# ISAE-PNX/SaDVIO

Measured on AMD Instinct MI355X. Metric: BA iterations/sec (ms/solve in ms_per_solve), 20-KF/8k-landmark window, higher is better.
Workload: dtype f64; 1 GPU; synthetic 20 KF x 8000 landmarks x 40000 reprojection factors (pixel), GN 10 iters (LM step attempts, early exits disabled); windows_per_gpu=1, parallelism=single window, n_kf=20, n_lmk=8000, n_obs=40000, reduced_dim=114

## Files before the change

sadvio_amd/csrc/ba_types.h:

```cpp
#pragma once
#include <stdint.h>

namespace sadvio {

struct SolveOpts {
    int max_num_iterations;
    int jacobi_scaling;
    int max_num_consecutive_invalid_steps;
    int pad;
    double function_tolerance, gradient_tolerance, parameter_tolerance;
    double initial_radius, max_radius, min_radius;
    double min_lm_diagonal, max_lm_diagonal, min_relative_decrease;
    double huber_a;
    double max_time_ticks;
};

struct WinDev {
    int n_kf, n_cam, n_lmk, n_obs;
    int kf_base, cam_base, lmk_base, obs_base;
    int n_free_kf, dpf, Np, Npose;
    long long S_off;
    int red_off;
    int tile_begin, tile_end;
    int prior_begin, prior_end;
// ... 80 lines not shown
    double radius, decrease_factor, x_cost, x_norm, initial_cost;
    int cur;
    int done, termination, iter;
    int n_success, n_unsuccess, n_invalid, pad;
};

struct FinalRec {
    LmState s;
    double fixed_cost;
};

struct IterAcc {
    double lin_cost;
    double cand_cost;
    double mcc;
    double step_norm2;
    double cand_norm2;
    double fixed_cost;
    unsigned long long gmax_bits;
    int chol_fail;
    int time_up;
};

struct TileAcc {
    double lin_cost, fixed_cost, gmax;
    double cand_cost, mcc, step_norm2, cand_norm2;
    double pad;
};

constexpr int BUILD_THREADS = 256;
constexpr int BUILD_WAVES = BUILD_THREADS / 64;
constexpr int MAX_TILE_KF = 24;
constexpr int MAX_TILE_FREE_KF = 20;
constexpr int MAX_GEMM_FREE_KF = 5;
constexpr int MAX_WIN_CAM = 8;
constexpr int STAGE_VALS = 18;
constexpr int MAX_LMK_OBS = 64;
constexpr int SOLVE_THREADS = 512;
constexpr int SOLVE_KFC_STRIDE = 32;
constexpr int SOLVE_KFC = 32;
constexpr int PRIOR_LIN = 28;
constexpr int PRE_KF = 8;
constexpr int PRE_MAX_TILES = 1024;
constexpr int MAX_LDS_NP = 174;

}
```

sadvio_amd/csrc/kernels.h:

```cpp
#pragma once
#include "ba_types.h"
#include "device_math.h"
#include "chol16.h"

namespace sadvio {

struct DevPtrs {
    const WinDev* win;
    const Tile* tiles;
    const double* kf_T0;
    const int* kf_fidx;
    double* xp; double* xv; double* xba; double* xbg;
    long long xp_stride, xv_stride, xl_stride;
    const double* kf_vel; const double* kf_ba; const double* kf_bg;
    const double* cam_K; const double* cam_T; const double* cam_isig;
    const double* lmk_p; double* xl; double* s_lmk;
    const unsigned char* lmk_const;
    const int* lmk_ob; const int* lmk_oe;
    const int* obs_kf; const int* obs_cam; const double* obs_meas;
    const unsigned char* obs_slot;
    const int* tile_kf;
    const int* tile_lmk;
    const int* tile_row;
    const int4* pre_lane;
// ... 421 lines not shown
    const Tile T = tiles[blockIdx.x];
    const int tid = threadIdx.x;
    if (tid < BUILD_THREADS / 8) {
        const int lane0 = tid * 8, wv = lane0 >> 6, ln = lane0 & 63;
        const int G = T.G, lpw = 64 / G, grp = ln / G, q0 = ln - grp * G, nl = T.n_lmk;
        const bool valid = wv * lpw + grp < nl;
        const int gl = nl > 0 ? tile_landmark(T, tile_lmk, valid ? wv * lpw + grp : 0) : T.lmk0;
        const int ob = nl > 0 ? lmk_ob[gl] : 0, nobs = (valid && nl > 0) ? lmk_oe[gl] - ob : 0;
        pre_lane[(long long)blockIdx.x * (BUILD_THREADS / 8) + tid] = make_int4(gl, ob, nobs | (valid ? 1 << 16 : 0), q0);
    }
    if (tid < PRE_KF) {
        int2 e = make_int2(-1, -1);
        if (tid < T.n_kf) { e.x = tile_kf[T.kf_off + tid]; e.y = kf_fidx[e.x]; }
        pre_kf[(long long)blockIdx.x * PRE_KF + tid] = e;
    }
}

template <bool COST_ONLY> __device__ __forceinline__ void pose_factor_eval(const DevPtrs& P, int slot, int idx, int ln);
template <int FACTOR, bool RARE, bool IMU>
__global__ __launch_bounds__(BUILD_THREADS, IMU ? 1 : 2) void k_build(DevPtrs P, int slot, int max_tile_kf, int strip_doubles, int Rp) {
    extern __shared__ __attribute__((aligned(16))) char smem[];
    if (IMU && (int)blockIdx.x >= P.n_tiles) {
        pose_factor_eval<false>(P, slot, (int)blockIdx.x - P.n_tiles, threadIdx.x);
        return;
    }
    const Tile T = P.tiles[blockIdx.x];
    const int tid = threadIdx.x, wv = tid >> 6, ln = tid & 63;
    int4 pl = make_int4(0, -1, 0, 0);
    int2 pk = make_int2(-1, -1);
    if (P.pre_lane) {
        pl = P.pre_lane[(long long)blockIdx.x * (BUILD_THREADS / 8) + (tid >> 3)];
        pk = P.pre_kf[(long long)blockIdx.x * PRE_KF + tid / POSE_TAB];
    }
    SADVIO_TS(3, 32);
    SADVIO_WG_TS(3, 0);
    __shared__ double s_part[BUILD_WAVES * 4];
    double* poseTab = (double*)smem;
    double* camTab = poseTab + (size_t)max_tile_kf * POSE_TAB;
    int* rowTab = (int*)(camTab + MAX_WIN_CAM * 17);
    double* stage = (double*)(smem + tile_tables_bytes(max_tile_kf));
    const int G = T.G, lpw = 64 / G;
    const int grp = ln / G, q = ln - grp * G;
    const int nl = T.n_lmk;
    LmState st;
    IterAcc a;
    LmState prev;
    const bool own_decision = !(slot == 0 || P.decide_kernel);
    double pc = 0.0, pm = 0.0, psn = 0.0, pcn = 0.0;
    auto decision_inputs = [&](int dec_w, int t0, int nt) {
        if (!own_decision) {
            st = P.states[(long long)dec_w * P.state_stride + slot];
            return;
        }
        a = P.acc[(long long)dec_w * P.state_stride + slot - 1];
        prev = P.states[(long long)dec_w * P.state_stride + slot - 1];
        if (P.world > 1) {
            if (wv == 0) {
                const double* rs = P.rank_s + (long long)dec_w * P.world * 4;
                for (int r = ln; r < P.world; r += 64) { pc += rs[4 * r]; pm += rs[4 * r + 1]; psn += rs[4 * r + 2]; pcn += rs[4 * r + 3]; }
            }
        } else {
            const TileAcc* ta = P.tacc + (long long)((slot - 1) & 1) * P.n_tiles + t0;
            double v[4][4];
#pragma unroll
            for (int u = 0; u < 4; u++) {
                const int t = tid + u * BUILD_THREADS;
                const bool in = t < nt;
                const TileAcc* e = ta + (in ? t : 0);
                v[u][0] = in ? e->cand_cost : 0.0; v[u][1] = in ? e->mcc : 0.0; v[u][2] = in ? e->step_norm2 : 0.0; v[u][3] = in ? e->cand_norm2 : 0.0;
            }
            pc = (v[0][0] + v[1][0]) + (v[2][0] + v[3][0]); pm = (v[0][1] + v[1][1]) + (v[2][1] + v[3][1]);
            psn = (v[0][2] + v[1][2]) + (v[2][2] + v[3][2]); pcn = (v[0][3] + v[1][3]) + (v[2][3] + v[3][3]);
        }
    };
    if (P.n_win == 1) decision_inputs(0, 0, P.n_tiles);
    else decision_inputs(T.w, T.win_tile0, T.win_ntiles);
    bool first_valid;
    int gl_first, pre_ob, pre_oe, pre_o;
    if (P.pre_lane) {
        first_valid = (pl.z >> 16) & 1; gl_first = pl.x; pre_ob = pl.y; pre_oe = pl.y + (pl.z & 0xff);
        pre_o = (pl.w + (tid & 7) < (pl.z & 0xff)) ? pl.y + pl.w + (tid & 7) : -1;
    } else {
        first_valid = wv * lpw + grp < nl;
        gl_first = tile_landmark(T, P.tile_lmk, first_valid ? wv * lpw + grp : 0);
        pre_ob = P.lmk_ob[gl_first]; pre_oe = P.lmk_oe[gl_first];
        pre_o = (first_valid && q < pre_oe - pre_ob) ? pre_ob + q : -1;
    }
    const int pre_lcode = P.lmk_const ? P.lmk_const[gl_first] : 0;
    double pre_p[3], pre_x0[3], pre_x1[3];
#pragma unroll
    for (int i = 0; i < 3; i++) {
        pre_p[i] = P.lmk_p[3 * (long long)gl_first + i];
        pre_x0[i] = P.xl[3 * (long long)gl_first + i];
        pre_x1[i] = P.xl[P.xl_stride + 3 * (long long)gl_first + i];
    }
    double pre_t0 = 0.0, pre_t1 = 0.0;
    if (P.pre_lane) {
        if (pk.x >= 0) {
            const long long src = (long long)pk.x * POSE_TAB + (tid - (tid / POSE_TAB) * POSE_TAB);
            pre_t0 = P.ptab[src]; pre_t1 = P.ptab[P.ptab_stride + src];
        }
    } else if (tid < T.n_kf * POSE_TAB) {
        const int k = tid / POSE_TAB, e = tid - k * POSE_TAB;
        const long long src = (long long)P.tile_kf[T.kf_off + k] * POSE_TAB + e;
        pre_t0 = P.ptab[src]; pre_t1 = P.ptab[P.ptab_stride + src];
    }
    for (int i = tid; i < T.n_cam * 17; i += blockDim.x) {
        const int c = i / 17, e = i - 17 * c;
        const int gc = T.cam_base + c;
        camTab[i] = e < 4 ? P.cam_K[4 * (long long)gc + e] : (e < 16 ? P.cam_T[12 * (long long)gc + e - 4] : P.cam_isig[gc]);
    }
    for (int i = tid; i < T.n_kf; i += blockDim.x) rowTab[i] = P.tile_row[T.kf_off + i];
    ObsPre pre_obs;
    pre_obs.slot = 0; pre_obs.craw = 0; pre_obs.m[0] = pre_obs.m[1] = pre_obs.m[2] = 0.0;
    if (pre_o >= 0) pre_obs = obs_prefetch<FACTOR>(P, pre_o);
    if (own_decision) {
        pc = wave_sum(pc); pm = wave_sum(pm); psn = wave_sum(psn); pcn = wave_sum(pcn);
        if (ln == 0) { s_part[wv * 4] = pc; s_part[wv * 4 + 1] = pm; s_part[wv * 4 + 2] = psn; s_part[wv * 4 + 3] = pcn; }
        __syncthreads();
        a.cand_cost += (s_part[0] + s_part[4]) + (s_part[8] + s_part[12]); a.mcc += (s_part[1] + s_part[5]) + (s_part[9] + s_part[13]);
        a.step_norm2 += (s_part[2] + s_part[6]) + (s_part[10] + s_part[14]); a.cand_norm2 += (s_part[3] + s_part[7]) + (s_part[11] + s_part[15]);
        st = lm_decide(prev, a, P.o);
        __syncthreads();
        if (T.first_of_window && tid == 0) { P.states[(long long)T.w * P.state_stride + slot] = st; trace_write(P, T.w, slot - 1, prev, a, st); }
    }
    if (st.done) return;
    SADVIO_TS(3, 33);
    double* Stile = stage + BUILD_WAVES * strip_doubles;
    const int Nt = 6 * T.n_free;
    const int tri_n = Nt * (Nt + 1) / 2;
    double* gT = Stile + tri_n;
    double* gfT = gT + Nt;
    double* hdT = gfT + Nt;
    const bool lds_mode = T.lds_mode != 0;
    if (tid < T.n_kf * POSE_TAB) poseTab[tid] = st.cur ? pre_t1 : pre_t0;
    {
        const double* src = P.ptab + (long long)st.cur * P.ptab_stride;
        for (int i = tid + blockDim.x; i < T.n_kf * POSE_TAB; i += blockDim.x) {
            const int k = i / POSE_TAB, e = i - k * POSE_TAB;
            poseTab[i] = src[(long long)P.tile_kf[T.kf_off + k] * POSE_TAB + e];
        }
    }
    if (lds_mode) {
        const int nz = tri_n + 3 * Nt;
        for (int i = tid; i < nz; i += blockDim.x) Stile[i] = 0.0;
    }
    __syncthreads();

    SADVIO_TS(3, 34);
    double* Sg = P.S + T.S_off;
    double* gredg = P.gred + T.red_off;
    double* gfullg = P.gfull + T.red_off;
    double* hdg = P.hdiag + T.red_off;
    const int dpf = T.dpf, Np = T.Np;
    const double* xl = P.xl + (long long)st.cur * P.xl_stride;
    double* wstage = stage + wv * strip_doubles;
    const bool gemm_mode = T.lds_mode == 2;
    double cost_part = 0.0, fixed_part = 0.0, gmax_part = 0.0;
    typedef double d4 __attribute__((ext_vector_type(4)));
    d4 accs[3] = {(d4){0.0, 0.0, 0.0, 0.0}, (d4){0.0, 0.0, 0.0, 0.0}, (d4){0.0, 0.0, 0.0, 0.0}};
    for (int base = wv * lpw; base < nl; base += BUILD_WAVES * lpw) {
        const int lm = base + grp;
        const bool lmk_valid = lm < nl;
        const bool first = base == wv * lpw;
        const int gl = first ? gl_first : tile_landmark(T, P.tile_lmk, lmk_valid ? lm : 0);
        const int ob = first ? pre_ob : P.lmk_ob[gl], oe = first ? pre_oe : P.lmk_oe[gl];
        const int nobs = lmk_valid ? oe - ob : 0;
        const int lcode = first ? pre_lcode : (P.lmk_const ? P.lmk_const[gl] : 0);
        const bool lfree = lcode == 0;
        ObsLin L;
        L.valid = q < nobs;
        L.row = -1; L.slot = 0; L.counted = false;
        if (L.valid) {
            double pw[3];
            ObsPre obq;
            if (first) {
#pragma unroll
                for (int i = 0; i < 3; i++) pw[i] = pre_p[i] + (st.cur ? pre_x1[i] : pre_x0[i]);
// ... 174 lines not shown
                    for (int j = 0; j < 6; j++) {
                        const int col = pb + j;
                        if (col > row) continue;
                        const double v = c0 * Jpb[j] + c1 * Jpb[6 + j];
                        if (lds_mode) atomic_add_f64(&Stile[tri(row, col)], v);
                        else atomic_add_f64(&Sg[s_index(T.ld, (pa / 6) * dpf + i, (pb / 6) * dpf + j)], v);
                    }
                }
            }
        }
        wave_lds_fence();
    }
        }
    if (gemm_mode && wv * lpw < nl) {
        const int lr = ln & 15, lk = ln >> 4;
        const int nt16 = (Nt + 15) >> 4;
#pragma unroll
        for (int pp = 0; pp < 3; pp++) {
            const int tr = pp < 1 ? 0 : 1, tc = pp - tr;
            if (tr < nt16) {
                const int col = 16 * tc + lr;
#pragma unroll
                for (int rg = 0; rg < 4; rg++) {
                    const int row = 16 * tr + lk + 4 * rg;
                    if (row < Nt && col <= row) atomic_add_f64(&Stile[tri(row, col)], -accs[pp][rg]);
                }
            }
        }
    }
    SADVIO_TS(3, 40);
    const double c = wave_sum(cost_part), f = wave_sum(fixed_part), gm = wave_max(gmax_part);
    if (ln == 0) { s_part[wv * 4] = c; s_part[wv * 4 + 1] = f; s_part[wv * 4 + 2] = gm; }
    __syncthreads();
    if (tid == 0) {
        double cs = 0.0, fs = 0.0, gs = 0.0;
        for (int k = 0; k < BUILD_WAVES; k++) { cs += s_part[k * 4]; fs += s_part[k * 4 + 1]; gs = fmax(gs, s_part[k * 4 + 2]); }
        TileAcc* ta = P.tacc + (long long)(slot & 1) * P.n_tiles + blockIdx.x;
        ta->lin_cost = cs; ta->fixed_cost = fs; ta->gmax = gs;
    }
    SADVIO_TS(3, 41);
    if (lds_mode) {
        int* growTab = (int*)stage;
        for (int k = tid; k < T.n_kf; k += blockDim.x) {
            const int r = rowTab[k];
            if (r >= 0) {
                const int fi = P.kf_fidx[P.tile_kf[T.kf_off + k]];
#pragma unroll
                for (int i = 0; i < 6; i++) growTab[r + i] = fi * dpf + i;
            }
        }
        __syncthreads();
        if (T.ld) {
            for (int row = wv; row < Nt; row += BUILD_WAVES) {
                const long long grow = (long long)growTab[row] * T.ld;
                const double* srow = Stile + tri(row, 0);
                for (int col = ln; col <= row; col += 64) {
                    const double v = srow[col];
                    if (v != 0.0) atomic_add_f64(&Sg[grow + growTab[col]], v);
                }
            }
        } else {
            for (int col = wv; col < Nt; col += BUILD_WAVES) {
                const int gc = growTab[col];
                for (int row = col + ln; row < Nt; row += 64) {
                    const double v = Stile[tri(row, col)];
                    if (v != 0.0) atomic_add_f64(&Sg[c16_index(growTab[row], gc)], v);
                }
            }
        }
        for (int i = tid; i < Nt; i += blockDim.x) {
            const int row = growTab[i];
            if (gT[i] != 0.0) atomic_add_f64(&gredg[row], gT[i]);
            if (gfT[i] != 0.0) atomic_add_f64(&gfullg[row], gfT[i]);
            if (hdT[i] != 0.0) atomic_add_f64(&hdg[row], hdT[i]);
        }
    }
    SADVIO_TS(3, 42);
    SADVIO_WG_TS(3, 1);
}

__device__ __forceinline__ double rsqrt_nr(double d) {
    double y = __builtin_amdgcn_rsq(d);
    const double t = d * y;
    const double e = __builtin_fma(-t, y, 1.0);
    const double p = __builtin_fma(0.375, e, 0.5);
    const double q = e * p;
    return __builtin_fma(y, q, y);
}

__device__ __forceinline__ double readlane_f64(double v, int lane) {
    int lo = __double2loint(v), hi = __double2hiint(v);
    lo = __builtin_amdgcn_readlane(lo, lane);
    hi = __builtin_amdgcn_readlane(hi, lane);
    return __hiloint2double(hi, lo);
}

constexpr int NBP = 6;

template <int NB>
__device__ __forceinline__ void factor_pivot(double (&Lk)[NB][NB], double (&Li)[NB][NB], bool& bad) {
#pragma unroll
    for (int j = 0; j < NB; j++) {
        double d = Lk[j][j];
#pragma unroll
        for (int q = 0; q < j; q++) d -= Lk[j][q] * Lk[j][q];
        if (!(d > 0.0) || !isfinite(d)) bad = true;
        double inv = rsqrt_nr(d);
        Lk[j][j] = d * inv;
        Li[j][j] = inv;
// ... 299 lines not shown
}

__device__ __noinline__ bool sparse_eval(const DevPtrs& P, const WinDev& W, const SparseDev& f, const double* xp, const double* xv,
                                        const double* xba, const double* xbg, const double* xl, const double* y,
                                        double* r, double* J) {
    return sparse_eval_t<false>(P, W, f, xp, xv, xba, xbg, xl, y, r, J);
}


__device__ __forceinline__ double prior_lin_record(const double* T0, const double* Tp, const double* inf, const double* d6, double* rec) {
    double r[6], J[36];
    pose_prior_factor(T0, Tp, inf, d6, r, J);
    double c = 0.0;
#pragma unroll
    for (int a = 0; a < 6; a++) {
        c += r[a] * r[a];
        double g = 0.0;
#pragma unroll
        for (int q = 0; q < 6; q++) g += J[6 * q + a] * r[q];
        rec[a] = g;
#pragma unroll
        for (int b = 0; b <= a; b++) {
            double hh = 0.0;
#pragma unroll
            for (int q = 0; q < 6; q++) hh += J[6 * q + a] * J[6 * q + b];
            rec[6 + a * (a + 1) / 2 + b] = hh;
        }
    }
    rec[27] = c;
    return c;
}

__device__ __noinline__ void pose_table_store(const double* T0, double d0, double d1, double d2, double d3, double d4, double d5, double* dst) {
    double T0r[12], tab[POSE_TAB];
#pragma unroll
    for (int i = 0; i < 12; i++) T0r[i] = T0[i];
    const double d6[6] = {d0, d1, d2, d3, d4, d5};
    pose_table_entry(T0r, d6, tab);
#pragma unroll
    for (int i = 0; i < POSE_TAB; i++) dst[i] = tab[i];
}
__device__ __noinline__ double prior_lin_record_call(const double* T0, double d0, double d1, double d2, double d3, double d4, double d5, const PriorDev* pr,
                                                     double* rec) {
    double T0r[12];
#pragma unroll
    for (int i = 0; i < 12; i++) T0r[i] = T0[i];
    const double d6[6] = {d0, d1, d2, d3, d4, d5};
    const PriorDev q = *pr;
    return prior_lin_record(T0r, q.T_prior, q.inf, d6, rec);
}

template <int MODE, bool EXTRAS>
__global__ __launch_bounds__(SOLVE_THREADS) void k_solve(DevPtrs P, int slot) {
    extern __shared__ __attribute__((aligned(16))) char smem[];
    constexpr bool BIG = MODE != 0;
    const int w = blockIdx.x;
    const WinDev W = P.win[w];
    if (BIG != (W.ld != 0)) return;
    const int tid = threadIdx.x;
    const int wv = __builtin_amdgcn_readfirstlane(tid >> 6), ln = tid & 63, nwv = blockDim.x >> 6;
    LmState* stp = P.states + (long long)w * P.state_stride + slot;
    IterAcc* acc = P.acc + (long long)w * P.state_stride + slot;
    __shared__ int s_done;
    __shared__ double s_red[SOLVE_THREADS / 64 * 4];
    SADVIO_TS(3, 0);
#ifdef SADVIO_KERNEL_TS
// ... 66 lines not shown
        c_y = gredg[tid]; c_gf = gfullg[tid]; c_hd = hdg[tid];
        if (slot != 0) c_sp = sp[tid];
    }
    const bool kf_pre = MODE == 0 && tid < W.n_kf && tid < SOLVE_KFC;
    int kf_fi = -1;
    double kf_t6[6], kf_t12[12], kf_vbb[9] = {0.0, 0.0, 0.0, 0.0, 0.0, 0.0, 0.0, 0.0, 0.0};
    if (kf_pre) {
        const int g = W.kf_base + tid;
        kf_fi = P.kf_fidx[g];
#pragma unroll
        for (int i = 0; i < 6; i++) kf_t6[i] = xp[6 * (long long)g + i];
#pragma unroll
        for (int i = 0; i < 12; i++) kf_t12[i] = P.kf_T0[12 * (long long)g + i];
        if (W.dpf == 15) {
            const double* xs3[3] = {P.xv + (long long)cur * P.xv_stride, P.xba + (long long)cur * P.xv_stride, P.xbg + (long long)cur * P.xv_stride};
#pragma unroll
            for (int q = 0; q < 3; q++)
#pragma unroll
                for (int i = 0; i < 3; i++) kf_vbb[3 * q + i] = xs3[q][3 * (long long)g + i];
        }
    }
    if (P.world > 1) {
        const double* rb = P.rank_b + (long long)w * P.world * 4;
        for (int r = tid; r < P.world; r += blockDim.x) { early_cost += rb[4 * r]; early_fixed += rb[4 * r + 1]; early_gm = fmax(early_gm, rb[4 * r + 2]); }
    } else {
        const TileAcc* ta = P.tacc + (long long)(slot & 1) * P.n_tiles + W.tile_begin;
        for (int t = tid; t < W.tile_end - W.tile_begin; t += blockDim.x) {
            early_cost += ta[t].lin_cost; early_fixed += ta[t].fixed_cost; early_gm = fmax(early_gm, ta[t].gmax);
        }
    }
    if (!BIG) {
        if (tid < Np) {
            y[tid] = c_y; gf[tid] = c_gf; hd[tid] = c_hd;
            gredg[tid] = 0.0; gfullg[tid] = 0.0; hdg[tid] = 0.0;
        }
        if (kf_pre) {
            double* c = kfc + tid * SOLVE_KFC_STRIDE;
            c[0] = (double)kf_fi;
#pragma unroll
            for (int i = 0; i < 6; i++) c[1 + i] = kf_t6[i];
#pragma unroll
            for (int i = 0; i < 12; i++) c[7 + i] = kf_t12[i];
            if (W.dpf == 15) {
#pragma unroll
                for (int i = 0; i < 9; i++) c[19 + i] = kf_vbb[i];
            }
        }
    }
    __syncthreads();
    SADVIO_TS(3, 1);
    if (det) {
        for (int p = 0; p < n_pri; p++) {
            const int fi = P.kf_fidx[P.priors[W.prior_begin + p].kf];
            if (tid < 28) {
                const double v = plin[p * PRIOR_LIN + tid];
                if (tid == 27) { if (fi < 0) fixed_part += v; else cost_part += v; }
                else if (fi >= 0) {
                    const int base = fi * W.dpf;
                    if (tid < 6) { y[base + tid] += v; gf[base + tid] += v; }
                    else {
                        const int q = tid - 6;
                        const int a = (int)((__builtin_sqrtf((float)(8 * q + 1)) - 1.0f) * 0.5f);
                        const int b = q - ((a * (a + 1)) >> 1);
                        A[aidx(base + a, base + b)] += v;
                        if (a == b) hd[base + a] += v;
                    }
                }
// ... 160 lines not shown
            if (slot == 0) { s = P.o.jacobi_scaling ? 1.0 / (1.0 + sqrt(hdi)) : 1.0; sp[tid] = s; }
            const double s2 = s * s;
            A[c16_index(tid, tid)] += fmin(fmax(s2 * hdi, P.o.min_lm_diagonal), P.o.max_lm_diagonal) / st.radius / s2;
            A[c16_index(Np, tid)] = y[tid];
        }
    } else {
        for (int i = tid; i < Np; i += blockDim.x) gm = fmax(gm, fabs(gf[i]));
    }
    gm = wave_max(gm); cost_part = wave_sum(cost_part); fixed_part = wave_sum(fixed_part);
    if (ln == 0) { s_red[wv * 3] = gm; s_red[wv * 3 + 1] = cost_part; s_red[wv * 3 + 2] = fixed_part; }
    if (tid == 0) s_done = 0;
    __syncthreads();
    if (!BIG) c16_symmetrize(A, nbt);
    if (tid == blockDim.x - 1) {
        double g = 0, cs = 0, fs = 0;
        for (int k = 0; k < nwv; k++) { g = fmax(g, s_red[k * 3]); cs += s_red[k * 3 + 1]; fs += s_red[k * 3 + 2]; }
        acc->gmax_bits = (unsigned long long)__double_as_longlong(g);
        acc->lin_cost = cs;
        acc->fixed_cost = fs;
        acc->cand_cost = 0.0; acc->mcc = 0.0; acc->step_norm2 = 0.0; acc->cand_norm2 = 0.0;
        const bool time_up = P.o.max_time_ticks > 0.0 && P.t_start && (double)(wall_clock64() - *P.t_start) >= P.o.max_time_ticks;
        acc->time_up = time_up ? 1 : 0;
        const bool no_iterations = st.iter == 0 && P.o.max_num_iterations <= 0;
        if (time_up || g <= P.o.gradient_tolerance || no_iterations) {
            LmState e = st;
            e.done = 1; e.termination = (time_up || g > P.o.gradient_tolerance) ? 0 : 3;
            e.x_cost = 0.5 * cs;
            if (e.iter == 0) e.initial_cost = e.x_cost;
            *stp = e;
            s_done = 1;
        }
    }
    __syncthreads();
    if (s_done) return;
    SADVIO_TS(3, 2);
    if (BIG) {
        for (int i = tid; i < Np; i += blockDim.x) {
            double s;
            if (slot == 0) { s = P.o.jacobi_scaling ? 1.0 / (1.0 + sqrt(hd[i])) : 1.0; sp[i] = s; }
            else s = sp[i];
            double s2 = s * s;
            A[aidx(i, i)] += fmin(fmax(s2 * hd[i], P.o.min_lm_diagonal), P.o.max_lm_diagonal) / st.radius / s2;
        }
        __syncthreads();
    }
    SADVIO_TS(3, 3);
    if (MODE == 1) return;
    }
    long long* ts = SADVIO_TS_PTR((P.debug & 4096) && blockIdx.x == 0 && slot == 3);
    if (MODE == 0) {
        bool ok = true;
        if (Np > 0) ok = c16_solve<1>(A, Np, xs, pub, yv, ts ? ts + 64 : nullptr);
        if (!ok) {
            if (tid == 0) acc->chol_fail = 1;
            return;
        }
    } else {
        y = P.delta + W.red_off;
        if (P.big_info[w] != 0) {
            for (int i = tid; i < Np; i += blockDim.x) { gredg[i] = 0.0; gfullg[i] = 0.0; hdg[i] = 0.0; }
            if (tid == 0) acc->chol_fail = 1;
            return;
        }
    }
    SADVIO_TS(3, 4);
    double* dl = P.delta + W.red_off;
    double sn = 0.0, cn = 0.0;
    bool bad = false;
    for (int i = tid; i < Np; i += blockDim.x) {
        double d = -xs[i];
        dl[i] = d;
        y[i] = d;
        sn += d * d;
        if (!isfinite(d)) bad = true;
        if (BIG) { gredg[i] = 0.0; gfullg[i] = 0.0; hdg[i] = 0.0; }
    }
    __syncthreads();
    SADVIO_TS(3, 5);
    double* xpc = P.xp + (long long)(1 - cur) * P.xp_stride;
    for (int k = tid; k < W.n_kf; k += blockDim.x) {
        int g = W.kf_base + k;
        const bool pre = MODE == 0 && k < SOLVE_KFC;
        const double* kc = kfc + (pre ? k : 0) * SOLVE_KFC_STRIDE;
        int fi = pre ? (int)kc[0] : P.kf_fidx[g];
        double d6[6];
        const double* T0r = pre ? kc + 7 : P.kf_T0 + 12 * (long long)g;
        double vbb[9];
        if (W.dpf == 15) {
            const double* xs3[3] = {P.xv + (long long)cur * P.xv_stride, P.xba + (long long)cur * P.xv_stride, P.xbg + (long long)cur * P.xv_stride};
#pragma unroll
            for (int q = 0; q < 3; q++)
#pragma unroll
                for (int i = 0; i < 3; i++) vbb[3 * q + i] = pre ? kc[19 + 3 * q + i] : xs3[q][3 * (long long)g + i];
        }
#pragma unroll
        for (int i = 0; i < 6; i++) {
            double v = (pre ? kc[1 + i] : xp[6 * (long long)g + i]) + (fi < 0 ? 0.0 : y[fi * W.dpf + i]);
            xpc[6 * (long long)g + i] = v;
            d6[i] = v;
            if (fi >= 0) cn += v * v;
        }
        pose_table_store(T0r, d6[0], d6[1], d6[2], d6[3], d6[4], d6[5], P.ptab + (long long)(1 - cur) * P.ptab_stride + (long long)g * POSE_TAB);
        if (W.dpf == 15) {
            double* xs3[3] = {P.xv + (long long)(1 - cur) * P.xv_stride, P.xba + (long long)(1 - cur) * P.xv_stride, P.xbg + (long long)(1 - cur) * P.xv_stride};
#pragma unroll
            for (int q = 0; q < 3; q++)
#pragma unroll
                for (int i = 0; i < 3; i++) {
                    const double v = vbb[3 * q + i] + (fi < 0 ? 0.0 : y[fi * 15 + 6 + 3 * q + i]);
                    xs3[q][3 * (long long)g + i] = v;
                    if (fi >= 0) cn += v * v;
                }
        }
// ... 70 lines not shown
            double jr[15], cd[15];
#pragma unroll
            for (int a = 0; a < 15; a++) { jr[a] = sc[q * 15 + a]; cd[a] = sc[SPARSE_COL + a]; }
            const double r = sc[225 + q];
            double m = 0.0;
#pragma unroll
            for (int a = 0; a < 15; a++) { const int ca = (int)cd[a]; if (ca >= 0) m += jr[a] * y[ca]; }
            mcc += -m * (r + 0.5 * m);
        }
    }
    if (EXTRAS && W.lobs_end > W.lobs_begin) {
        const int rows = W.factor_type == 0 ? 4 : 2;
        for (int it = tid; it < (W.lobs_end - W.lobs_begin) * 4; it += blockDim.x) {
            const int k = it >> 2, q = it & 3;
            if (q >= rows) continue;
            const LineObsDev& ob = P.lobs[W.lobs_begin + k];
            const int fi = P.kf_fidx[ob.kf], lc = P.lines[ob.line].col;
            if (fi < 0 && lc < 0) continue;
            const double* sc = P.line_scratch + (long long)(W.lobs_begin + k) * LINE_ROW;
            double m = 0.0;
            for (int a = 0; a < 6; a++) {
                if (fi >= 0) m += sc[q * 12 + a] * y[fi * W.dpf + a];
                if (lc >= 0) m += sc[q * 12 + 6 + a] * y[lc + a];
            }
            mcc += -m * (sc[48 + q] + 0.5 * m);
        }
    }
    SADVIO_TS(3, 7);
    sn = wave_sum(sn); cn = wave_sum(cn); mcc = wave_sum(mcc); cc = wave_sum(cc);
    if (bad) acc->chol_fail = 1;
    __syncthreads();
    if (ln == 0) { s_red[wv * 4] = sn; s_red[wv * 4 + 1] = cn; s_red[wv * 4 + 2] = mcc; s_red[wv * 4 + 3] = cc; }
    __syncthreads();
    if (tid == 0) {
        double a0 = 0, a1 = 0, a2 = 0, a3 = 0;
        for (int k = 0; k < nwv; k++) { a0 += s_red[k * 4]; a1 += s_red[k * 4 + 1]; a2 += s_red[k * 4 + 2]; a3 += s_red[k * 4 + 3]; }
        acc->step_norm2 = a0; acc->cand_norm2 = a1; acc->mcc = a2; acc->cand_cost = a3;
    }
    SADVIO_TS(3, 8);
    if (ts && tid == 0) { ts[15] = wall_clock64(); ts[21] = clock64(); }
}


__device__ __forceinline__ void zero_s_slice(const DevPtrs& P, const Tile& T, int tile_index) {
    if (T.ld != 0) return;
    const int n2 = c16_size(T.Np) >> 1;
    const int per = (n2 + T.win_ntiles - 1) / T.win_ntiles;
    const int i0 = (tile_index - T.win_tile0) * per, i1 = min(i0 + per, n2);
    double2* S2 = (double2*)(P.S + T.S_off);
    const double2 z2 = make_double2(0.0, 0.0);
    for (int i = i0 + (int)threadIdx.x; i < i1; i += blockDim.x) S2[i] = z2;
}

template <int FACTOR, bool RARE, bool IMU>
__global__ __launch_bounds__(BUILD_THREADS) void k_backsub(DevPtrs P, int slot, int max_tile_kf) {
    extern __shared__ __attribute__((aligned(16))) char smem[];
    if (IMU && (int)blockIdx.x >= P.n_tiles) {
        if (threadIdx.x < 64) pose_factor_eval<true>(P, slot, (int)blockIdx.x - P.n_tiles, threadIdx.x);
        return;
    }
    const Tile T = P.tiles[blockIdx.x];
    const int tid = threadIdx.x, wv = tid >> 6, ln = tid & 63;
    int4 pl = make_int4(0, -1, 0, 0);
    int2 pk = make_int2(-1, -1), pk6 = make_int2(-1, -1);
    if (P.pre_lane) {
        pl = P.pre_lane[(long long)blockIdx.x * (BUILD_THREADS / 8) + (tid >> 3)];
// ... 1117 lines not shown
```

sadvio_amd/csrc/solve_driver.h:

```cpp
#pragma once
#include <cstddef>
#include <type_traits>

#include "ba_handle.h"

namespace {

DevPtrs make_ptrs(sadvio_ba_handle* h, const SolveOpts& o, int state_stride) {
    DevPtrs P{};
    P.win = h->d_win.p; P.tiles = h->d_tiles.p;
    P.kf_T0 = h->d_kf_T0.p; P.kf_fidx = h->d_kf_fidx.p;
    P.xp = h->d_xp.p; P.xv = h->d_xv.p; P.xba = h->d_xba.p; P.xbg = h->d_xbg.p;
    P.xp_stride = 6LL * h->n_kf_tot; P.xv_stride = 3LL * h->n_kf_tot; P.xl_stride = 3LL * h->n_lmk_tot;
    P.kf_vel = h->d_kf_vel.p; P.kf_ba = h->d_kf_ba.p; P.kf_bg = h->d_kf_bg.p;
    P.cam_K = h->d_cam_K.p; P.cam_T = h->d_cam_T.p; P.cam_isig = h->d_cam_isig.p;
    P.lmk_p = h->d_lmk_p.p; P.xl = h->d_xl.p; P.s_lmk = h->d_s_lmk.p;
    P.lmk_const = h->has_lmk_const ? h->d_lmk_const.p : nullptr;
    P.lmk_ob = h->d_lmk_ob.p; P.lmk_oe = h->d_lmk_oe.p;
    P.obs_kf = h->d_obs_kf.p; P.obs_cam = h->d_obs_cam.p; P.obs_meas = h->d_obs_meas.p;
    P.obs_slot = h->d_obs_slot.p; P.tile_kf = h->d_tile_kf.p; P.tile_lmk = h->d_tile_lmk.p; P.tile_row = h->d_tile_row.p;
    P.pre_lane = h->pre_ok ? (const int4*)h->d_pre_lane.p : nullptr; P.pre_kf = h->pre_ok ? (const int2*)h->d_pre_kf.p : nullptr;
    P.ptab = h->d_ptab.p; P.ptab_stride = (long long)POSE_TAB * h->n_kf_tot;
    P.priors = h->d_priors.p; P.prior_lin = h->d_prior_lin.p; P.prior_lin_stride = (long long)h->priors.size() * PRIOR_LIN; P.n_prior_tot = (int)h->priors.size();
    P.imus = h->d_imus.p; P.imu_scratch = h->d_imu_scratch.p; P.imu_scratch_stride = (long long)h->imus.size() * IMU_ROW;
// ... 211 lines not shown

int plan_solve(sadvio_ba_handle* h, const SolveOpts& o, SolvePlan& plan, std::vector<BigPlan>& big) {
    memset(&plan, 0, sizeof(plan));
    const int n_win = (int)h->wins.size();
    const int slots = plan.slots = std::max(1, o.max_num_iterations);
    const int stride = slots + 2;
    HIP_TRY(h->d_dbg.alloc(DBG_SLOTS));
    HIP_TRY(h->d_states.alloc((size_t)n_win * stride));
    HIP_TRY(h->d_trace.alloc((size_t)n_win * stride * 8));
    HIP_TRY(h->d_tstart.alloc(1));
    HIP_TRY(h->d_acc.alloc((size_t)n_win * stride));
    HIP_TRY(h->d_final.alloc((size_t)n_win));
    HIP_TRY(h->d_big_info.alloc((size_t)n_win));
    if (h->h_final_n < (size_t)n_win) {
        if (h->h_final) (void)hipHostFree(h->h_final);
        h->h_final = nullptr; h->h_final_n = 0;
        HIP_TRY(hipHostMalloc((void**)&h->h_final, sizeof(FinalRec) * (size_t)n_win, hipHostMallocDefault));
        h->h_final_n = (size_t)n_win;
    }
    DevPtrs& P = plan.P;
    P = make_ptrs(h, o, stride);
    const int n_tiles = (int)h->tiles.size();
    int max_win_tiles = 0;
    for (int w = 0; w < n_win; w++) max_win_tiles = std::max(max_win_tiles, h->wins[w].d.tile_end - h->wins[w].d.tile_begin);
    plan.max_win_tiles = max_win_tiles;
    P.decide_kernel = max_win_tiles > 4 * BUILD_THREADS ? 1 : 0;
    P.imu_direct = (!h->coll_fn && P.world == 1 && !h->env.imu_items) ? 1 : 0;
    const int mtk = plan.mtk = h->max_tile_kf;
    const size_t nt = 6 * (size_t)h->max_tile_free;
    int Rp = 16 * ((6 * h->max_gemm_free + 15) / 16);
    int strip_doubles = std::max(STAGE_VALS * 64, 2 * Rp * (32 + 2));
    size_t lds_build = tile_tables_bytes(mtk) + sizeof(double) * ((size_t)BUILD_WAVES * strip_doubles + nt * (nt + 1) / 2 + 3 * nt +
                                                                   0) + 16;
    if (lds_build > 160 * 1024 && h->max_gemm_free > 0) {
        for (auto& t : h->tiles) if (t.lds_mode == 2) t.lds_mode = 1;
        HIP_TRY(hipMemcpyAsync(h->d_tiles.p, h->tiles.data(), h->tiles.size() * sizeof(Tile), hipMemcpyHostToDevice, h->stream));
        h->max_gemm_free = 0;
        Rp = 0; strip_doubles = STAGE_VALS * 64;
        lds_build = tile_tables_bytes(mtk) + sizeof(double) * ((size_t)BUILD_WAVES * strip_doubles + nt * (nt + 1) / 2 + 3 * nt +
                                                               0) + 16;
    }
    if (h->env.debug) fprintf(stderr, "[sadvio dbg] lds_build %zu B, Rp %d, strip_doubles %d, max_tile_kf %d, max_tile_free %d, tiles %d\n", lds_build, Rp, strip_doubles, mtk, h->max_tile_free, n_tiles);
    plan.Rp = Rp; plan.strip_doubles = strip_doubles; plan.lds_build = lds_build;
    plan.lds_back = tile_tables_bytes(mtk) + sizeof(double) * ((size_t)mtk * 18) + 16;
    const size_t npq = (size_t)h->max_np;
    plan.lds_solve = sizeof(double) * ((size_t)c16_size((int)npq) + 4 * npq + 1 + C16_WORK + 16 * (size_t)c16_blocks((int)npq + 1) + SOLVE_KFC * SOLVE_KFC_STRIDE) + 64;
    bool any_pseudo = false;
    for (const auto& v : h->sp_elim) for (char e : v) any_pseudo |= e != 0;
    bool any_kept_lmk = false;
    for (int w = 0; w < n_win; w++) any_kept_lmk |= h->wins[w].d.n_red > 0;
    const bool rare = plan.rare = o.huber_a > 0.0 || h->n_kept > 0 || any_kept_lmk || any_pseudo || h->gemm_run4;
    const bool pix = plan.pix = h->factor_type == SADVIO_FACTOR_PIXEL;
    const bool have_pf = !h->imus.empty() || h->n_sp_list > 0;
    bool with_imu = have_pf && n_tiles <= 3 * 256;
    if (h->env.pf_wg >= 0) with_imu = have_pf && h->env.pf_wg != 0;
    plan.with_imu = with_imu;
    plan.k_build = build_variant(pix, rare, with_imu);
    plan.k_backsub = backsub_variant(pix, rare, with_imu);
    plan.k_build_kept = pix ? k_build_kept<0> : k_build_kept<1>;
    bool use_lm = h->lm_ok && !rare && !h->coll_fn && h->world == 1 && h->lm_landmarks >= 65536;
    if (h->env.lm >= 0) use_lm = h->lm_ok && !rare && !h->coll_fn && h->world == 1 && h->env.lm != 0;
    plan.use_lm = use_lm;
    plan.k_build_obs = pix ? k_build_obs<0> : k_build_obs<1>;
    plan.k_lm_pass = pix ? k_lm_pass<0, false> : k_lm_pass<1, false>;
    plan.k_lm_pass0 = pix ? k_lm_pass<0, true> : k_lm_pass<1, true>;
    plan.lm_n_sub = h->lm_n_sub; plan.lm_sub_obs = h->lm_sub_obs;
    const size_t lds_views = pix ? sizeof(double) * (size_t)mtk * h->lm_max_cam * LM_VT : 0;
// ... 214 lines not shown
```

Measured before the change: 18490 BA iterations/s.

## Hoist build-kernel row table setup, defer state writes, and stage solve pose tables in LDS

In the build kernel, the global row-index table is now computed early into a static shared array using prefetched keyframe indices. This replaces a late loop with dependent global loads and an extra barrier. The LM state write and the per-tile accumulator write are moved to the kernel tail so they no longer sit on the critical path. In the solve kernel's MODE 0 update, pose tables are computed into LDS and then written to global memory with vectorized coalesced stores, parked parameters are flushed in bulk, and gradient zeroing is moved after a barrier. The cost is more static LDS, accounted for in the LDS budget check, plus added code complexity.

```diff
diff --git a/sadvio_amd/csrc/ba_types.h b/sadvio_amd/csrc/ba_types.h
--- a/sadvio_amd/csrc/ba_types.h
+++ b/sadvio_amd/csrc/ba_types.h
@@ -136,6 +136,7 @@
 constexpr int BUILD_WAVES = BUILD_THREADS / 64;
 constexpr int MAX_TILE_KF = 24;
 constexpr int MAX_TILE_FREE_KF = 20;
+constexpr int BUILD_STATIC_LDS = 4 * 6 * MAX_TILE_FREE_KF + 512;
 constexpr int MAX_GEMM_FREE_KF = 5;
 constexpr int MAX_WIN_CAM = 8;
 constexpr int STAGE_VALS = 18;
diff --git a/sadvio_amd/csrc/kernels.h b/sadvio_amd/csrc/kernels.h
--- a/sadvio_amd/csrc/kernels.h
+++ b/sadvio_amd/csrc/kernels.h
@@ -477,9 +477,13 @@
         pl = P.pre_lane[(long long)blockIdx.x * (BUILD_THREADS / 8) + (tid >> 3)];
         pk = P.pre_kf[(long long)blockIdx.x * PRE_KF + tid / POSE_TAB];
     }
+    int2 gk = make_int2(-1, -1);
+    const bool gk_pre = P.pre_lane && tid < PRE_KF;
+    if (gk_pre) gk = P.pre_kf[(long long)blockIdx.x * PRE_KF + tid];
     SADVIO_TS(3, 32);
     SADVIO_WG_TS(3, 0);
     __shared__ double s_part[BUILD_WAVES * 4];
+    __shared__ int growTab[6 * MAX_TILE_FREE_KF];
     double* poseTab = (double*)smem;
     double* camTab = poseTab + (size_t)max_tile_kf * POSE_TAB;
     int* rowTab = (int*)(camTab + MAX_WIN_CAM * 17);
@@ -491,6 +495,9 @@
     IterAcc a;
     LmState prev;
     const bool own_decision = !(slot == 0 || P.decide_kernel);
+    const bool st_writer = own_decision && T.first_of_window && tid == 0;
+    __shared__ LmState s_dec[2];
+    __shared__ IterAcc s_dec_a;
     double pc = 0.0, pm = 0.0, psn = 0.0, pcn = 0.0;
     auto decision_inputs = [&](int dec_w, int t0, int nt) {
         if (!own_decision) {
@@ -556,9 +563,11 @@
         camTab[i] = e < 4 ? P.cam_K[4 * (long long)gc + e] : (e < 16 ? P.cam_T[12 * (long long)gc + e - 4] : P.cam_isig[gc]);
     }
     for (int i = tid; i < T.n_kf; i += blockDim.x) rowTab[i] = P.tile_row[T.kf_off + i];
+    if (T.lds_mode != 0 && !gk_pre && tid < T.n_kf) gk.x = P.tile_kf[T.kf_off + tid];
     ObsPre pre_obs;
     pre_obs.slot = 0; pre_obs.craw = 0; pre_obs.m[0] = pre_obs.m[1] = pre_obs.m[2] = 0.0;
     if (pre_o >= 0) pre_obs = obs_prefetch<FACTOR>(P, pre_o);
+    if (T.lds_mode != 0 && !gk_pre && tid < T.n_kf) gk.y = P.kf_fidx[gk.x];
     if (own_decision) {
         pc = wave_sum(pc); pm = wave_sum(pm); psn = wave_sum(psn); pcn = wave_sum(pcn);
         if (ln == 0) { s_part[wv * 4] = pc; s_part[wv * 4 + 1] = pm; s_part[wv * 4 + 2] = psn; s_part[wv * 4 + 3] = pcn; }
@@ -567,7 +576,10 @@
         a.step_norm2 += (s_part[2] + s_part[6]) + (s_part[10] + s_part[14]); a.cand_norm2 += (s_part[3] + s_part[7]) + (s_part[11] + s_part[15]);
         st = lm_decide(prev, a, P.o);
         __syncthreads();
-        if (T.first_of_window && tid == 0) { P.states[(long long)T.w * P.state_stride + slot] = st; trace_write(P, T.w, slot - 1, prev, a, st); }
+        if (st_writer) {
+            if (IMU || st.done) { P.states[(long long)T.w * P.state_stride + slot] = st; trace_write(P, T.w, slot - 1, prev, a, st); }
+            else { s_dec[0] = prev; s_dec[1] = st; s_dec_a = a; }
+        }
     }
     if (st.done) return;
     SADVIO_TS(3, 33);
@@ -589,6 +601,13 @@
     if (lds_mode) {
         const int nz = tri_n + 3 * Nt;
         for (int i = tid; i < nz; i += blockDim.x) Stile[i] = 0.0;
+        if (tid < T.n_kf) {
+            const int r = rowTab[tid];
+            if (r >= 0) {
+#pragma unroll
+                for (int i = 0; i < 6; i++) growTab[r + i] = gk.y * T.dpf + i;
+            }
+        }
     }
     __syncthreads();
 
@@ -829,24 +848,8 @@
     const double c = wave_sum(cost_part), f = wave_sum(fixed_part), gm = wave_max(gmax_part);
     if (ln == 0) { s_part[wv * 4] = c; s_part[wv * 4 + 1] = f; s_part[wv * 4 + 2] = gm; }
     __syncthreads();
-    if (tid == 0) {
-        double cs = 0.0, fs = 0.0, gs = 0.0;
-        for (int k = 0; k < BUILD_WAVES; k++) { cs += s_part[k * 4]; fs += s_part[k * 4 + 1]; gs = fmax(gs, s_part[k * 4 + 2]); }
-        TileAcc* ta = P.tacc + (long long)(slot & 1) * P.n_tiles + blockIdx.x;
-        ta->lin_cost = cs; ta->fixed_cost = fs; ta->gmax = gs;
-    }
     SADVIO_TS(3, 41);
     if (lds_mode) {
-        int* growTab = (int*)stage;
-        for (int k = tid; k < T.n_kf; k += blockDim.x) {
-            const int r = rowTab[k];
-            if (r >= 0) {
-                const int fi = P.kf_fidx[P.tile_kf[T.kf_off + k]];
-#pragma unroll
-                for (int i = 0; i < 6; i++) growTab[r + i] = fi * dpf + i;
-            }
-        }
-        __syncthreads();
         if (T.ld) {
             for (int row = wv; row < Nt; row += BUILD_WAVES) {
                 const long long grow = (long long)growTab[row] * T.ld;
@@ -872,6 +875,13 @@
             if (hdT[i] != 0.0) atomic_add_f64(&hdg[row], hdT[i]);
         }
     }
+    if (tid == 0) {
+        double cs = 0.0, fs = 0.0, gs = 0.0;
+        for (int k = 0; k < BUILD_WAVES; k++) { cs += s_part[k * 4]; fs += s_part[k * 4 + 1]; gs = fmax(gs, s_part[k * 4 + 2]); }
+        TileAcc* ta = P.tacc + (long long)(slot & 1) * P.n_tiles + blockIdx.x;
+        ta->lin_cost = cs; ta->fixed_cost = fs; ta->gmax = gs;
+    }
+    if (!IMU && st_writer) { P.states[(long long)T.w * P.state_stride + slot] = s_dec[1]; trace_write(P, T.w, slot - 1, s_dec[0], s_dec_a, s_dec[1]); }
     SADVIO_TS(3, 42);
     SADVIO_WG_TS(3, 1);
 }
@@ -1237,6 +1247,16 @@
 }
 
 __device__ __noinline__ void pose_table_store(const double* T0, double d0, double d1, double d2, double d3, double d4, double d5, double* dst) {
+    double T0r[12], tab[POSE_TAB];
+#pragma unroll
+    for (int i = 0; i < 12; i++) T0r[i] = T0[i];
+    const double d6[6] = {d0, d1, d2, d3, d4, d5};
+    pose_table_entry(T0r, d6, tab);
+#pragma unroll
+    for (int i = 0; i < POSE_TAB; i++) dst[i] = tab[i];
+}
+typedef __attribute__((address_space(3))) double lds_double_t;
+__device__ __noinline__ void pose_table_lds(const lds_double_t* T0, double d0, double d1, double d2, double d3, double d4, double d5, lds_double_t* dst) {
     double T0r[12], tab[POSE_TAB];
 #pragma unroll
     for (int i = 0; i < 12; i++) T0r[i] = T0[i];
@@ -1369,7 +1389,6 @@
     if (!BIG) {
         if (tid < Np) {
             y[tid] = c_y; gf[tid] = c_gf; hd[tid] = c_hd;
-            gredg[tid] = 0.0; gfullg[tid] = 0.0; hdg[tid] = 0.0;
         }
         if (kf_pre) {
             double* c = kfc + tid * SOLVE_KFC_STRIDE;
@@ -1596,6 +1615,7 @@
         }
     }
     __syncthreads();
+    if (!BIG && tid < Np) { gredg[tid] = 0.0; gfullg[tid] = 0.0; hdg[tid] = 0.0; }
     if (s_done) return;
     SADVIO_TS(3, 2);
     if (BIG) {
@@ -1642,7 +1662,92 @@
     __syncthreads();
     SADVIO_TS(3, 5);
     double* xpc = P.xp + (long long)(1 - cur) * P.xp_stride;
-    for (int k = tid; k < W.n_kf; k += blockDim.x) {
+    lds_double_t* Al = (lds_double_t*)(double*)smem;
+    lds_double_t* yl = Al + img_n;
+    lds_double_t* kfcl = Al + (kfc - (double*)smem);
+    const int tab_cap = img_n / POSE_TAB;
+    for (int k = tid; MODE == 0 && k < W.n_kf; k += blockDim.x) {
+        const int g = W.kf_base + k;
+        const bool staged = k < tab_cap;
+        lds_double_t* kc = kfcl + (k < SOLVE_KFC ? k : 0) * SOLVE_KFC_STRIDE;
+        lds_double_t* tdst = Al + (staged ? k : 0) * POSE_TAB;
+        const lds_double_t* T0l = kc + 7;
+        int fi;
+        double x6[6], vbb[9], dy[15];
+        if (k < SOLVE_KFC) {
+            fi = (int)kc[0];
+#pragma unroll
+            for (int i = 0; i < 6; i++) x6[i] = kc[1 + i];
+            if (W.dpf == 15) {
+#pragma unroll
+                for (int i = 0; i < 9; i++) vbb[i] = kc[19 + i];
+            }
+        } else {
+            fi = P.kf_fidx[g];
+#pragma unroll
+            for (int i = 0; i < 6; i++) x6[i] = xp[6 * (long long)g + i];
+            if (W.dpf == 15) {
+                const double* xs3[3] = {P.xv + (long long)cur * P.xv_stride, P.xba + (long long)cur * P.xv_stride, P.xbg + (long long)cur * P.xv_stride};
+#pragma unroll
+                for (int q = 0; q < 3; q++)
+#pragma unroll
+                    for (int i = 0; i < 3; i++) vbb[3 * q + i] = xs3[q][3 * (long long)g + i];
+            }
+            if (staged) {
+                double t12[12];
+#pragma unroll
+                for (int i = 0; i < 12; i++) t12[i] = P.kf_T0[12 * (long long)g + i];
+#pragma unroll
+                for (int i = 0; i < 12; i++) tdst[i] = t12[i];
+                T0l = tdst;
+            }
+        }
+#pragma unroll
+        for (int i = 0; i < 6; i++) dy[i] = fi < 0 ? 0.0 : yl[fi * W.dpf + i];
+        if (W.dpf == 15) {
+#pragma unroll
+            for (int i = 0; i < 9; i++) dy[6 + i] = fi < 0 ? 0.0 : yl[fi * 15 + 6 + i];
+        }
+        double d6[6];
+#pragma unroll
+        for (int i = 0; i < 6; i++) {
+            const double v = x6[i] + dy[i];
+            d6[i] = v;
+            if (fi >= 0) cn += v * v;
+        }
+        if (W.dpf == 15) {
+#pragma unroll
+            for (int i = 0; i < 9; i++) {
+                const double v = vbb[i] + dy[6 + i];
+                vbb[i] = v;
+                if (fi >= 0) cn += v * v;
+            }
+        }
+        if (k < SOLVE_KFC) {
+#pragma unroll
+            for (int i = 0; i < 6; i++) kc[1 + i] = d6[i];
+            if (W.dpf == 15) {
+#pragma unroll
+                for (int i = 0; i < 9; i++) kc[19 + i] = vbb[i];
+            }
+        }
+        if (staged) pose_table_lds(T0l, d6[0], d6[1], d6[2], d6[3], d6[4], d6[5], tdst);
+        else
+            pose_table_store(k < SOLVE_KFC ? (const double*)(kfc + k * SOLVE_KFC_STRIDE + 7) : P.kf_T0 + 12 * (long long)g, d6[0], d6[1], d6[2], d6[3], d6[4], d6[5],
+                             P.ptab + (long long)(1 - cur) * P.ptab_stride + (long long)g * POSE_TAB);
+        if (k >= SOLVE_KFC) {
+#pragma unroll
+            for (int i = 0; i < 6; i++) xpc[6 * (long long)g + i] = d6[i];
+            if (W.dpf == 15) {
+                double* xs3[3] = {P.xv + (long long)(1 - cur) * P.xv_stride, P.xba + (long long)(1 - cur) * P.xv_stride, P.xbg + (long long)(1 - cur) * P.xv_stride};
+#pragma unroll
+                for (int q = 0; q < 3; q++)
+#pragma unroll
+                    for (int i = 0; i < 3; i++) xs3[q][3 * (long long)g + i] = vbb[3 * q + i];
+            }
+        }
+    }
+    for (int k = tid; MODE != 0 && k < W.n_kf; k += blockDim.x) {
         int g = W.kf_base + k;
         const bool pre = MODE == 0 && k < SOLVE_KFC;
         const double* kc = kfc + (pre ? k : 0) * SOLVE_KFC_STRIDE;
@@ -1779,6 +1884,25 @@
     __syncthreads();
     if (ln == 0) { s_red[wv * 4] = sn; s_red[wv * 4 + 1] = cn; s_red[wv * 4 + 2] = mcc; s_red[wv * 4 + 3] = cc; }
     __syncthreads();
+    if (MODE == 0) {
+        typedef double d2v __attribute__((ext_vector_type(2)));
+        typedef __attribute__((address_space(3))) d2v lds_d2v_t;
+        const int n_tab = min(W.n_kf, tab_cap), n_park = min(W.n_kf, SOLVE_KFC);
+        d2v* pt2 = (d2v*)(P.ptab + (long long)(1 - cur) * P.ptab_stride + (long long)W.kf_base * POSE_TAB);
+        const lds_d2v_t* A2l = (const lds_d2v_t*)Al;
+        for (int i = tid; i < n_tab * (POSE_TAB / 2); i += blockDim.x) pt2[i] = A2l[i];
+        for (int i = (int)blockDim.x - 1 - tid; i < n_park * 6; i += blockDim.x) {
+            const int k = i / 6, e = i - 6 * k;
+            xpc[6 * (long long)W.kf_base + i] = kfcl[k * SOLVE_KFC_STRIDE + 1 + e];
+        }
+        if (W.dpf == 15) {
+            for (int i = (int)blockDim.x - 1 - tid; i < n_park * 9; i += blockDim.x) {
+                const int k = i / 9, e = i - 9 * k, q = e / 3;
+                double* b = (q == 0 ? P.xv : q == 1 ? P.xba : P.xbg) + (long long)(1 - cur) * P.xv_stride;
+                b[3 * (long long)(W.kf_base + k) + (e - 3 * q)] = kfcl[k * SOLVE_KFC_STRIDE + 19 + e];
+            }
+        }
+    }
     if (tid == 0) {
         double a0 = 0, a1 = 0, a2 = 0, a3 = 0;
         for (int k = 0; k < nwv; k++) { a0 += s_red[k * 4]; a1 += s_red[k * 4 + 1]; a2 += s_red[k * 4 + 2]; a3 += s_red[k * 4 + 3]; }
diff --git a/sadvio_amd/csrc/solve_driver.h b/sadvio_amd/csrc/solve_driver.h
--- a/sadvio_amd/csrc/solve_driver.h
+++ b/sadvio_amd/csrc/solve_driver.h
@@ -267,7 +267,7 @@
     int strip_doubles = std::max(STAGE_VALS * 64, 2 * Rp * (32 + 2));
     size_t lds_build = tile_tables_bytes(mtk) + sizeof(double) * ((size_t)BUILD_WAVES * strip_doubles + nt * (nt + 1) / 2 + 3 * nt +
                                                                    0) + 16;
-    if (lds_build > 160 * 1024 && h->max_gemm_free > 0) {
+    if (lds_build + BUILD_STATIC_LDS > 160 * 1024 && h->max_gemm_free > 0) {
         for (auto& t : h->tiles) if (t.lds_mode == 2) t.lds_mode = 1;
         HIP_TRY(hipMemcpyAsync(h->d_tiles.p, h->tiles.data(), h->tiles.size() * sizeof(Tile), hipMemcpyHostToDevice, h->stream));
         h->max_gemm_free = 0;
```

New measurement: 18530 BA iterations/s, median of 4. Within noise of the previous version (+0.2%).
